# mittinatten/freesasa

Measured on AMD Instinct MI355X. Metric: atoms/sec SASA (L&R 20 slices), higher is better.
Workload: dtype f64

## Files before the change

### freesasa_amd/csrc/lr2_kernels.h

```cpp
#ifndef LR2_KERNELS_H
#define LR2_KERNELS_H

#include "sasa_kernels.h"

#ifdef SASA_EMU
namespace sasa_emu {
unsigned long long wave_ballot(bool p);
void wave_sync();
long long wave_exchange(long long v, int src);
}
#define LR2_BALLOT(p) sasa_emu::wave_ballot(p)
#define LR2_SYNC() sasa_emu::wave_sync()
#define LR2_SHFL(v, src) ((int)sasa_emu::wave_exchange((long long)(v), (src)))
#define LR2_POPC64(m) __builtin_popcountll(m)
#define LR2_POPC32(m) __builtin_popcount(m)
#define LR2_RANK(m, lane) __builtin_popcountll((m) & ((1ull << (lane)) - 1ull))
#define LR2_SHIFT_IN_LT1(w, c) (((w) << 1) | ((c) < 1.0 ? 1u : 0u))
#define LR2_SHIFT_IN_LT(w, v, lim) (((w) << 1) | ((v) < (lim) ? 1u : 0u))
#define LR2_UNIFORM(v) (v)
#define LR2_READLANE(v, src) LR2_SHFL((v), (src))
#define LR2_MUL24(a, b) ((int)(a) * (int)(b))
#define LR2_UMUL24(a, b) ((unsigned)(a) * (unsigned)(b))
#define LR2_RCPF(x) (1.0f / (x))
#define LR2_RSQF(x) (1.0f / sqrtf(x))
// ... 181 lines not shown
#define LR2_WARM(a, field) ((a).field)
#else
#define LR2_COLD(a, field) (*(const decltype(sasa::Lr2Args::field) *)lr2_cold_arg(offsetof(sasa::Lr2Args, field)))
#define LR2_WARM(a, field) LR2_COLD(a, field)
__device__ __forceinline__ const char *lr2_cold_arg(size_t off)
{
    auto p = __builtin_amdgcn_kernarg_segment_ptr();
    asm volatile("" : "+s"(p));
    return (const char *)p + off;
}
#endif

struct __attribute__((aligned(16))) Ab16 { double a, b; };
struct __attribute__((aligned(16))) Arc2 { double s, e; };

struct Lr2Layout {
    int o_atoms, o_ints, o_rec, o_mask, o_queue, o_tc, o_r2, o_tag, total;
};
SASA_HD int lr2_a16(int v) { return (v + 15) & ~15; }
SASA_HD int lr2_n_ints(int TA, int mw) { return 6 * TA + 1 + 8 + TA * mw; }
SASA_HD int lr2_n_row_ints(int TA) { return 9 * TA + 9 * TA + (9 * TA + 2); }
SASA_HD Lr2Layout lr2_layout(int TA, int ns, int pool, int mw, int ds)
{
    Lr2Layout L;
    const int items = TA * ns;
    int p = 0;
    L.o_atoms = p; p += 32 * TA + lr2_a16(8 * TA);
    L.o_ints = p;  p += lr2_a16(4 * lr2_n_ints(TA, mw));
    L.o_rec = p;   p += lr2_a16(24 * pool);
    L.o_mask = p;  p += lr2_a16(4 * items * mw);
    L.o_queue = p; p += lr2_a16(2 * items);
    L.o_tc = p;    p += lr2_a16(8 * items);
    if (p - L.o_rec < 32 * pool) p = L.o_rec + 32 * pool;
    int r2k = lr2_a16(8 * pool);
    if (r2k < lr2_a16(4 * lr2_n_row_ints(TA))) r2k = lr2_a16(4 * lr2_n_row_ints(TA));
    int r2 = r2k + lr2_a16(pool);
    const int r2q = lr2_a16(2 * items) + 256, r2s = 16 * LR2_LANES * (ds > 0 ? ds : 1);
    if (r2q > r2) r2 = r2q;
    if (r2s > r2) r2 = r2s;
    L.o_r2 = p;
    L.o_tag = p + r2k;
    p += r2;
    L.total = p;
    return L;
}

struct Lr2Mem {
    Quad *atom;
    double *adel;
    int *acell, *lead, *gsz, *acnt, *aoff, *sorig, *flags, *hist;
    unsigned *cmask;
    int *rowlo, *rinfo, *cpre;
    double *it_tc;
    unsigned *it_mask;
    unsigned short *queue;
    unsigned short *qtmp;
    Quad *hits;
    Ab16 *ab;
    double *beta;
    double *keys;
    unsigned char *tag;
    Arc2 *stack;
};

template <int SHAPE = 0>
SASA_D Lr2Mem lr2_carve(const Lr2Args &a, char *smem)
{
    const Lr2Layout L = lr2_layout(LR2_A_TA(a), LR2_A_NS(a), a.pool, LR2_A_MW(a), LR2_A_DS(a));
    const int TA = LR2_A_TA(a);
    Lr2Mem m;
    m.atom = (Quad *)(smem + L.o_atoms); m.adel = (double *)(smem + L.o_atoms + 32 * TA);
    int *q = (int *)(smem + L.o_ints);
    m.acell = q; q += TA; m.lead = q; q += TA; m.gsz = q; q += TA; m.acnt = q; q += TA; m.aoff = q; q += TA + 1;
    m.sorig = q; q += TA; m.flags = q; q += 8;
    m.cmask = (unsigned *)q;
    m.rowlo = (int *)(smem + L.o_r2); m.rinfo = m.rowlo + 9 * TA; m.cpre = m.rinfo + 9 * TA;
    m.it_tc = (double *)(smem + L.o_tc);
    m.it_mask = (unsigned *)(smem + L.o_mask);
    m.queue = (unsigned short *)(smem + L.o_queue);
    m.hits = (Quad *)(smem + L.o_rec);
    m.ab = (Ab16 *)(smem + L.o_rec);
    m.beta = (double *)(smem + L.o_rec + 16 * a.pool);
    m.keys = (double *)(smem + L.o_r2);
    m.tag = (unsigned char *)(smem + L.o_tag);
    m.hist = (int *)(smem + L.o_r2);
    m.qtmp = (unsigned short *)(smem + L.o_r2 + 256);
    m.stack = (Arc2 *)(smem + L.o_r2);
    return m;
}

SASA_D void lr2_record(double xd, double yd, double zd, double rj, double ri, double &ap, double &bp, double &Kout, double &d3sq, double &inv_d)
{
    const double D = xd * xd + yd * yd;
    double h;
    LR2_H2(D, h);
    const double inv = D > 0 ? 2.0 * h : 0x1p500;
    inv_d = D > 0 ? inv : 0.0;
    d3sq = D + zd * zd;
    const double K = (ri * ri - rj * rj) + d3sq;
    Kout = K;
    ap = -2.0 * zd * inv;
    bp = K * inv;
    if (!(D > 0) && zd == 0 && K == 0) bp = NAN;
}

SASA_D double lr2_arc_alpha(double t, const Ab16 &ab, double hh)
{
    const double v = fma(t, ab.a, ab.b);
    return acos_fast2_z(fma(fabs(v), -hh, 0.5), v);
}

struct Lr2Union {
    double ts, te, bs, be;
    int depth;
};
SASA_D void lr2_union_reset(Lr2Union &u) { u.ts = 0; u.te = -INFINITY; u.bs = 0; u.be = -INFINITY; u.depth = 0; }
SASA_D int lr2_med3(int v, int lo, int hi)
{
#ifdef SASA_EMU
    return v < lo ? lo : (v > hi ? hi : v);
#else
    int r;
    asm("v_med3_i32 %0, %1, %2, %3" : "=v"(r) : "v"(v), "s"(lo), "v"(hi));
    return r;
#endif
}
SASA_D Arc2 &lr2_level(Arc2 *stk, int depth, int ds)
{
    return (stk - 2 * LR2_LANES)[lr2_med3(depth, 2, ds > 0 ? ds + 1 : 2) * LR2_LANES];
}
SASA_D void lr2_union_step(double inf, double sup, Lr2Union &u, Arc2 *stk, int ds, int &maxd)
{
#ifdef LR2_UNION_SELECT
    const bool fresh = inf > u.te;
    const double mts = SASA_MIN(u.ts, inf), mte = SASA_MAX(u.te, sup);
    if (fresh) {
        Arc2 t; t.s = u.bs; t.e = u.be;
        lr2_level(stk, u.depth, ds) = t;
        u.bs = u.ts; u.be = u.te;
    }
    u.ts = fresh ? inf : mts;
    u.te = fresh ? sup : mte;
    u.depth += fresh ? 1 : 0;
    maxd = maxd > u.depth ? maxd : u.depth;
    while (u.be >= u.ts) {
        u.ts = SASA_MIN(u.ts, u.bs);
        --u.depth;
        if (u.depth >= 2) {
            const Arc2 lo = lr2_level(stk, u.depth, ds);
            u.bs = lo.s; u.be = lo.e;
        } else {
            u.be = -INFINITY;
        }
    }
#else
    if (inf > u.te) {
        Arc2 t; t.s = u.bs; t.e = u.be;
        lr2_level(stk, u.depth, ds) = t;
        u.bs = u.ts; u.be = u.te;
        u.ts = inf; u.te = sup;
        ++u.depth;
        maxd = maxd > u.depth ? maxd : u.depth;
    } else {
        u.ts = SASA_MIN(u.ts, inf);
        u.te = SASA_MAX(u.te, sup);
        while (u.be >= u.ts) {
            u.ts = SASA_MIN(u.ts, u.bs);
            --u.depth;
            if (u.depth >= 2) {
                const Arc2 lo = lr2_level(stk, u.depth, ds);
                u.bs = lo.s; u.be = lo.e;
            } else {
                u.be = -INFINITY;
            }
        }
    }
#endif
}

SASA_D double lr2_sweep(const Lr2Union &u, const Arc2 *stk, int ds)
{
    const int depth = u.depth;
    const bool two = depth >= 2;
    double s0 = two ? u.bs : u.ts;
    double e_below = two ? u.be : INFINITY;
    double sum = 0;
    if (depth > 2) {
        const Arc2 k0 = stk[0];
        s0 = k0.s;
        const double hi_ = s0 + SASA_TWOPI, lo_ = u.te - SASA_TWOPI;
        double pe = k0.e;
        for (int c = 1; c < depth - 2; ++c) {
            const Arc2 k = stk[(c < ds ? c : 0) * LR2_LANES];
            sum += SASA_MAX(SASA_MIN(k.s, hi_) - SASA_MAX(pe, lo_), 0.0);
            pe = k.e;
        }
        sum += SASA_MAX(SASA_MIN(u.bs, hi_) - SASA_MAX(pe, lo_), 0.0);
    }
    const double hi = s0 + SASA_TWOPI, lo = u.te - SASA_TWOPI;
    sum += SASA_MAX(SASA_MIN(u.ts, hi) - SASA_MAX(e_below, lo), 0.0);
    sum += SASA_MAX(hi - u.te, 0.0);
    return depth == 0 ? SASA_TWOPI : sum;
}

SASA_D double lr2_arc_kat(const double *arcs, const int *first, int k, Arc2 *stk, int ds)
{
    Lr2Union u;
    lr2_union_reset(u);
    int maxd = 0;
    for (int i = first[k]; i < first[k + 1]; ++i) lr2_union_step(arcs[2 * i], arcs[2 * i + 1], u, stk, ds, maxd);
    return maxd - 2 > ds ? NAN : lr2_sweep(u, stk, ds);
}

#ifndef LR2_NB_UNROLL
#ifndef LR2_ARC_STEPS
#define LR2_ARC_STEPS 2
#endif
#define LR2_NB_UNROLL 1
#endif
#define LR2_P1_G 3
#ifndef LR2_P1_G_COILS
#define LR2_P1_G_COILS LR2_P1_G
#endif
#define LR2_P1_G_OF(shape) ((shape) == 4 ? 4 : ((shape) == 1 ? LR2_P1_G_COILS : LR2_P1_G))
#define LR2_P1_HC(gs, g) ((g) == 4 ? ((gs) + 3) >> 2 : ((g) == 2 ? ((gs) + 1) >> 1 : lr2_div3((gs) + 2)))
#ifndef LR2_P1_ITEMS_MAX
#define LR2_P1_ITEMS_MAX 0x8000
#endif

SASA_D void lr2_overflow(const Lr2Args &a, int p0, int na, int err_code)
{
    int *const ovf_atoms = LR2_COLD(a, ovf_atoms), *const ovf_count = LR2_COLD(a, ovf_count);
    long long *const ovf_items = LR2_COLD(a, ovf_items);
    if (ovf_atoms) {
        const int w = SASA_ATOMIC_ADD_GLB(ovf_count, na);
        for (int k = 0; k < na; ++k) ovf_atoms[w + k] = p0 + k;
    } else if (ovf_items) {
        const int w = SASA_ATOMIC_ADD_GLB(ovf_count, 1);
        ovf_items[w] = (long long)p0 | ((long long)na << 32);
    } else {
        SASA_ATOMIC_MAX_GLB(&LR2_COLD(a, status)[ST_ERROR], err_code);
    }
}


SASA_D double lr2_slice_height(int s, double delta, double Ri) { return fma((double)s + 0.5, delta, -Ri); }
#ifndef LR2_WALK_Z
#define LR2_WALK_Z 1024.0
#endif
template <bool WALK>
SASA_D double lr2_slice_height_at(int s, double delta, double Ri, double zi)
{
    if (!WALK || !(fabs(zi) > LR2_WALK_Z)) return lr2_slice_height(s, delta, Ri);
    double z = (zi - Ri) - 0.5 * delta;
    for (int k = 0; k <= s; ++k) z += delta;
    return z - zi;
}

SASA_D unsigned lr2_tie12(double xd, double yd, double zd)
{
    unsigned long long a, b, c;
    memcpy(&a, &xd, 8); memcpy(&b, &yd, 8); memcpy(&c, &zd, 8);
    const unsigned h = (unsigned)a ^ ((unsigned)b * 0x9E3779B1u) ^ ((unsigned)c >> 7) ^ ((unsigned)c << 11);
    return (h ^ (h >> 13)) & 0xfffu;
}

#ifndef LR2_COVER_WANT
#define LR2_COVER_WANT 12
#endif
#define LR2_COVER_DENSITY 30
#ifndef LR2_COVER_MAX
#define LR2_COVER_MAX 20
#endif
SASA_D int lr2_cover_bin(double K, double d3sq, double ri)
{
    const float ct = (float)K * LR2_RSQF((float)d3sq) * LR2_RCPF(2.0f * (float)ri);
    const int b = (int)fmaf(ct, 10.0f, -2.0f);
    return b < 0 ? 0 : (b > 7 ? 7 : b);
}
SASA_D int lr2_cover_last_bin(unsigned long long h)
{
    int cum = 0, tb = 7;
    for (int b = 0; b < 8; ++b) {
        cum += (int)((h >> (8 * b)) & 255u);
        if (cum >= LR2_COVER_WANT && b < tb) tb = b;
    }
    return tb;
}
SASA_D double lr2_acos_lower(double c)
{
    const double c2 = c * c, k5 = c < 0 ? 0.075 : 0.17;
    return (1.5707963267948966 - 1e-9) - fma(c * c2, fma(k5, c2, 1.0 / 6.0), c);
}

#ifndef LR2_PRUNE
#define LR2_PRUNE 1
#endif
#ifndef LR2_PRUNE_ROUNDS
#define LR2_PRUNE_ROUNDS(pairs) ((pairs) ? 3 : 2)
#endif
#ifndef LR2_PRUNE_LIST
#define LR2_PRUNE_LIST 4
#endif
#define LR2_DEAD_TAG 0xff
struct __attribute__((aligned(16))) Lr2Cap { float x, y, z, c; };
SASA_HD int lr2_prune_arg(int want, int TA, int pool)
{
    if (8 * pool < (16 + 20 * LR2_PRUNE_LIST) * 2 * TA) return 0;
    return want > LR2_PRUNE_LIST ? LR2_PRUNE_LIST : (want < 0 ? 0 : want);
}
static inline int lr2_prune_want(int ns, bool dense) { return ns >= 32 ? 4 : (dense ? 0 : 3); }
SASA_D int lr2_cap_bin(float c) { const int b = (int)fmaf(c, 10.0f, -2.0f); return b < 0 ? 0 : (b > 7 ? 7 : b); }
template <int RMAX>
SASA_D void lr2_prune_contained(const Lr2Mem &m, int nh, int TA, int want, int lane)
{
    constexpr int LK = LR2_PRUNE_LIST;
    (void)want;
    unsigned long long *const chist = (unsigned long long *)m.keys;
    Lr2Cap *const bigc = (Lr2Cap *)(chist + 2 * TA);
    Lr2Cap *const bigs = bigc + 2 * LK * TA;
    int *const fill = m.acell;
    if (lane < 2 * TA) { chist[lane] = 0; fill[lane] = 0; }
    LR2_SYNC();
    float nx[RMAX], ny[RMAX], nz[RMAX], cc[RMAX];
    int lis[RMAX];
#define LR2_CAP_SIN(c) LR2_SQRTF(fmaf(-(c), (c), 1.0f + 4e-6f))
#define LR2_CAP_LIST(r, gp) ((gp) < nh && ny[r] != 0.0f && ny[r] == ny[r] ? 2 * (int)m.tag[gp] + (ny[r] > 0.0f ? 1 : 0) : -1)
    for (int r = 0; r < RMAX; ++r) {
        const int gp = lane + LR2_LANES * r;
        nx[r] = ny[r] = nz[r] = cc[r] = 0.0f;
        lis[r] = -1;
        if (gp < nh) {
            const Quad hq = m.hits[gp];
            const double ri = m.atom[(int)m.tag[gp]].w;
            const double d2 = hq.x * hq.x + hq.y * hq.y + hq.z * hq.z;
            const double K = (ri * ri - hq.w * hq.w) + d2;
            const float inv = LR2_RSQF((float)d2);
            nx[r] = (float)hq.x * inv; ny[r] = (float)hq.y * inv; nz[r] = (float)hq.z * inv;
            float c = (float)K * inv * LR2_RCPF(2.0f * (float)ri);
            c = c < -1.0f ? -1.0f : (c > 1.0f ? 1.0f : c);
            cc[r] = c;
            const int li = lis[r] = LR2_CAP_LIST(r, gp);
            if (li >= 0) LR2_ADD64_LDS(&chist[li], 1ull << (8 * lr2_cap_bin(c)));
        }
    }
    LR2_SYNC();
    if (lane < 2 * TA) {
        const unsigned long long h = chist[lane];
        const unsigned lo = (unsigned)h * 0x01010101u, hi = (unsigned)(h >> 32) * 0x01010101u + (lo >> 24) * 0x01010101u;
        const unsigned add = (unsigned)(127 - LK) * 0x01010101u;
        const unsigned mlo = (lo + add) & 0x80808080u, mhi = (hi + add) & 0x80808080u;
        const int tb = (mlo ? __builtin_ctz(mlo) >> 3 : (mhi ? 4 + (__builtin_ctz(mhi) >> 3) : 8)) - 1;
        chist[lane] = (unsigned long long)(long long)tb;
    }
    LR2_SYNC();
    for (int r = 0; r < RMAX; ++r) {
        const int li = lis[r];
        if (li < 0) continue;
        if (lr2_cap_bin(cc[r]) <= (int)chist[li]) {
            const int slot = SASA_ATOMIC_ADD_LDS(&fill[li], 1);
            if (slot < LK) {
                Lr2Cap q; q.x = nx[r]; q.y = ny[r]; q.z = nz[r]; q.c = cc[r];
                bigc[LK * li + slot] = q;
                ((float *)bigs)[LK * li + slot] = LR2_CAP_SIN(cc[r]);
            }
        }
    }
    LR2_SYNC();
    for (int r = 0; r < RMAX; ++r) {
        const int gp = lane + LR2_LANES * r;
        const int li = lis[r];
        if (li < 0) continue;
        const Lr2Cap *const L = bigc + LK * li;
        const float *const S = (const float *)bigs + LK * li;
        const float clim = cc[r] - 4e-6f, sj = LR2_CAP_SIN(cc[r]);
        bool inside = false;
        int nb = fill[li];
        nb = nb < LK ? nb : LK;
        for (int k = 0; k < nb; ++k) {
            const Lr2Cap q = L[k];
            const float dot = fmaf(nz[r], q.z, fmaf(ny[r], q.y, nx[r] * q.x));
            const float rhs = fmaf(sj, S[k], fmaf(cc[r], q.c, 8e-6f));
            inside = inside || (q.c <= clim && dot >= rhs);
        }
        if (inside) {
            m.tag[gp] = (unsigned char)LR2_DEAD_TAG;
            SASA_ATOMIC_ADD_LDS(&m.acnt[li >> 1], -1);
        }
    }
#undef LR2_CAP_LIST
#undef LR2_CAP_SIN
    LR2_SYNC();
}

struct Lr2Pre {
    int p0;
    long long rcf;
    int s0, s1;
    unsigned long long w0, w1;
    int rfl;
    Quad q;
    int cell, so;
};
SASA_D void lr2_pre_none(Lr2Pre &pre)
{
    pre.p0 = -1; pre.rcf = 0; pre.s0 = pre.s1 = 0; pre.w0 = pre.w1 = 0; pre.rfl = 1; pre.cell = 0; pre.so = 0;
    pre.q.x = pre.q.y = pre.q.z = 0; pre.q.w = 1;
}
template <int SHAPE>
SASA_D void lr2_pre_a(const Lr2Args &a, Lr2Pre &pre, int p0, int na, int lane)
{
    const int la = lr2_div9(lane);
    pre.p0 = p0;
    pre.rcf = LR2_WARM(a, s_idx)[p0 + (la < na ? la : na - 1)].cell;
}
template <int SHAPE>
SASA_D void lr2_pre_b(const Lr2Args &a, Lr2Pre &pre, int na, int lane)
{
    const int la = lr2_div9(lane), r = lane - 9 * la;
    const int c = (int)(pre.rcf & 0xffffffffLL), hw = (int)(pre.rcf >> 32);
    const int cprev = LR2_SHFL(c, lane >= 9 ? lane - 9 : lane);
    const int fl = hw & 63;
    int nx = (hw >> 6) & 8191, ny = (hw >> 19) & 8191;
    if (nx == 0) {
        const GridS *const g = LR2_COLD(a, grid) + LR2_COLD(a, s_idx)[pre.p0 + (la < na ? la : na - 1)].strct;
        nx = g->nx; ny = g->ny;
        SASA_OPAQUE(nx); SASA_OPAQUE(ny);
    }
    const int dz = lr2_div3(r < 9 ? r : 0) - 1, dy = (r < 9 ? r : 0) - 3 * (dz + 1) - 1;
    const bool out = (dy < 0 && (fl & CELL_Y0)) || (dy > 0 && (fl & CELL_Y1)) ||
                     (dz < 0 && (fl & CELL_Z0)) || (dz > 0 && (fl & CELL_Z1));
    const int row = out ? c : c + nx * (dy + ny * dz);
    const int x_lo = row - ((fl & CELL_X0) ? 0 : 1), x_hi = row + ((fl & CELL_X1) ? 0 : 1);
    const unsigned long long *const tbl = LR2_WARM(a, cell_tbl);
    if (tbl) {
        pre.s0 = x_lo; pre.s1 = x_hi + 1;
        pre.w0 = tbl[x_lo >> 5]; pre.w1 = tbl[(x_hi + 1) >> 5];
    } else {
        const int *const cell_start = LR2_COLD(a, cell_start);
        pre.s0 = cell_start[x_lo]; pre.s1 = cell_start[x_hi + 1];
    }
    pre.rfl = (out || la >= na ? 1 : 0) | (la == 0 || cprev != c ? 2 : 0);
}
template <int SHAPE>
SASA_D void lr2_pre_b2(const Lr2Args &a, Lr2Pre &pre)
{
    if (!LR2_WARM(a, cell_tbl)) return;
    const int *const first = LR2_WARM(a, cell_first);
    const int r0 = cell_rank(pre.w0, pre.s0), r1 = cell_rank(pre.w1, pre.s1);
    pre.s0 = first[r0]; pre.s1 = first[r1];
}
template <int SHAPE>
SASA_D void lr2_pre_c(const Lr2Args &a, Lr2Pre &pre, int na, int lane)
{
    const int p = pre.p0 + (lane < na ? lane : na - 1);
    pre.q = a.sq[p];
    const SortIdx si = LR2_WARM(a, s_idx)[p];
    pre.cell = lane < na ? (int)(si.cell & 0xffffffffLL) : -1 - lane;
    pre.so = si.orig;
}

template <int RMAX, bool COVER, bool PAIRS, int SHAPE, bool HOOKS, bool WALK>
SASA_D int lr2_tile(const Lr2Args &a, const Lr2Mem &m, int p0, int na, bool sample, bool tie_by_place, int lane_of_wave, int &wg_max_nn,
                    Lr2Pre &pre, int p0n, int nan, int &far_tiles)
{
    int lane = lane_of_wave;
    if (COVER) SASA_OPAQUE(lane);
    const int TA = LR2_A_TA(a), ns = LR2_A_NS(a), mw = LR2_A_MW(a);
    const int items = na * ns;
    LR2_MARK_BEGIN;
    LR2_COUNT(0, 1);

    if (pre.p0 != p0) {
        LR2_COUNT(11, 1);
        pre.p0 = p0;
        lr2_pre_c<SHAPE>(a, pre, na, lane);
        lr2_pre_a<SHAPE>(a, pre, p0, na, lane);
        lr2_pre_b<SHAPE>(a, pre, na, lane);
        lr2_pre_b2<SHAPE>(a, pre);
    }
    if (!HOOKS && (!WALK || !a.work_items) && LR2_BALLOT(lane < na && fabs(pre.q.z) > LR2_WALK_Z) != 0) {
        ++far_tiles;
        if (!WALK) {
            lr2_pre_none(pre);
            return 3;
        }
    }
    if (lane < TA) {
        Quad q = pre.q;
        if (lane >= na) { q.x = q.y = q.z = 0; q.w = 1; }
        const double del = lane < na ? lr2_div_ns(2 * q.w, (double)ns, LR2_WARM(a, inv_ns)) : 0.0;
        m.atom[lane] = q; m.adel[lane] = del; m.sorig[lane] = lane < na ? pre.so : 0;
        m.acnt[lane] = 0;
        m.gsz[lane] = 0;
    }
    if (lane < 8) m.flags[lane] = 0;
    unsigned lm;
    {
        const int cprev = LR2_SHFL(pre.cell, lane > 0 ? lane - 1 : 0);
        lm = (unsigned)LR2_BALLOT(lane < na && (lane == 0 || pre.cell != cprev));
    }
    int lo = 0, my_cnt = 0, info = 0;
    {
        const int la = lr2_div9(lane);
        if (la < na && (pre.rfl & 3) == 2) {
            const unsigned above = lm >> (la + 1);
            const int gs = (above ? la + 1 + __builtin_ctz(above) : na) - la, hc = LR2_P1_HC(gs, LR2_P1_G_OF(SHAPE));
            lo = pre.s0;
            my_cnt = LR2_MUL24(pre.s1 - pre.s0, hc);
            info = la | (gs << 4) | (hc << 8) | ((hc == 1 ? 0x20000 : (hc == 2 ? 0x10000 : 0xaaab)) << 10);
        }
    }
    lr2_pre_none(pre);
    const unsigned long long rm = LR2_BALLOT(my_cnt > 0);
    const int incl = lr2_scan_add(my_cnt, lane);
    const int nrows = LR2_POPC64(rm);
    const int total_c = LR2_READLANE(incl, LR2_LANES - 1);
    if (lane == 0) m.cpre[0] = 0;
    if (my_cnt > 0) {
        const int ri = LR2_RANK(rm, lane);
        m.cpre[ri + 1] = incl; m.rowlo[ri] = lo; m.rinfo[ri] = info;
    }
    LR2_SYNC();
    if (total_c >= LR2_P1_ITEMS_MAX) { LR2_COUNT(9, 1); return 1; }

    LR2_STOP(0);
    LR2_MARK(0);
    int nh = 0;
    {
        const int per = (total_c + LR2_LANES - 1) / LR2_LANES;
        const int f = lane * per;
        const int fend = f + per < total_c ? f + per : total_c;
        int t = 0;
        int c_lo = 0, c_hi = 0, rl = 0, ri_ = 0;
        if (f < total_c) {
            for (int step = 32; step >= 1; step >>= 1)
                if (t + step <= nrows - 1 && m.cpre[t + step] <= f) t += step;
            c_lo = m.cpre[t]; c_hi = m.cpre[t + 1]; rl = m.rowlo[t]; ri_ = m.rinfo[t];
        }
        constexpr int P1_G = LR2_P1_G_OF(SHAPE);
        LR2_COUNT(3, (per + LR2_NB_UNROLL - 1) / LR2_NB_UNROLL * LR2_NB_UNROLL * P1_G);
        for (int base = 0; base < per; base += LR2_NB_UNROLL) {
            int q[LR2_NB_UNROLL], la0[LR2_NB_UNROLL], two[LR2_NB_UNROLL];
            double x[LR2_NB_UNROLL], y[LR2_NB_UNROLL], z[LR2_NB_UNROLL], rq[LR2_NB_UNROLL];
            for (int j = 0; j < LR2_NB_UNROLL; ++j) {
                const int fj = f + base + j;
                const bool live = fj < fend;
                if (live && fj >= c_hi) {
                    ++t;
                    c_lo = c_hi; c_hi = m.cpre[t + 1]; rl = m.rowlo[t]; ri_ = m.rinfo[t];
                }
                const int lead = ri_ & 15, gs = (ri_ >> 4) & 15, hc = (ri_ >> 8) & 3;
                const unsigned i = (unsigned)(fj - c_lo) & 0x7fffu;
                const unsigned c = LR2_UMUL24(i, (unsigned)ri_ >> 10) >> 17;
                const int h = (int)i - LR2_MUL24(c, hc);
                const int left = gs - P1_G * h;
                q[j] = live ? rl + (int)c : -1;
                la0[j] = live ? lead + P1_G * h : 0;
                two[j] = live ? (left < P1_G ? left : P1_G) : 0;
            }
            for (int j = 0; j < LR2_NB_UNROLL; ++j) {
                const unsigned u = (unsigned)(q[j] < 0 ? 0 : q[j]);
                { const Quad v = a.sq[u]; x[j] = v.x; y[j] = v.y; z[j] = v.z; rq[j] = v.w; }
            }
            for (int g = 0; g < P1_G; ++g) {
                bool hit[LR2_NB_UNROLL];
                double dx[LR2_NB_UNROLL], dy[LR2_NB_UNROLL], dz[LR2_NB_UNROLL];
                Quad ai[LR2_NB_UNROLL];
                for (int j = 0; j < LR2_NB_UNROLL; ++j) ai[j] = m.atom[la0[j] + (g < two[j] ? g : 0)];
                for (int j = 0; j < LR2_NB_UNROLL; ++j) {
                    const double cut2 = (ai[j].w + rq[j]) * (ai[j].w + rq[j]);
                    dx[j] = x[j] - ai[j].x; dy[j] = y[j] - ai[j].y; dz[j] = z[j] - ai[j].z;
                    const double d2 = dx[j] * dx[j] + dy[j] * dy[j] + dz[j] * dz[j];
                    hit[j] = (g < two[j]) & (q[j] != p0 + la0[j] + g) & (d2 < cut2);
                }
                for (int j = 0; j < LR2_NB_UNROLL; ++j) {
                    const unsigned long long hm = LR2_BALLOT(hit[j]);
                    if (hit[j]) {
                        const int la = la0[j] + g;
                        int slot = nh + LR2_RANK(hm, lane);
                        slot = slot < a.pool ? slot : a.pool - 1;
                        Quad hq; hq.x = dx[j]; hq.y = dy[j]; hq.z = dz[j]; hq.w = rq[j];
                        m.hits[slot] = hq;
                        m.tag[slot] = (unsigned char)la;
                        if (!(HOOKS && (a.hooks & 2))) {
                            LR2_INC_LDS(&m.acnt[la]);
                        } else {
                            const int sa = SASA_ATOMIC_ADD_LDS(&m.acnt[la], 1);
                            const int cap = LR2_COLD(a, nb_cap);
                            if (sa < cap) LR2_COLD(a, nb_out)[(size_t)m.sorig[la] * cap + sa] = LR2_COLD(a, s_idx)[q[j]].orig;
                        }
                    }
                    nh += LR2_POPC64(hm);
                }
            }
        }
    }
    LR2_SYNC();

    LR2_STOP(1);
    LR2_MARK(1);
    if (HOOKS && (a.hooks & 1)) {
        if (lane < na) LR2_COLD(a, nn_out)[m.sorig[lane]] = m.acnt[lane];
        LR2_SYNC();
        return 0;
    }
    bool ovf;
    int nn_max;
    {
        const int c = lane < TA ? m.acnt[lane] : 0, pc = (c + 1) & ~1;
        const int incl = lr2_scan_add(pc, lane), cmax = lr2_scan_max16(c, lane);
        if (lane < TA) m.aoff[lane] = incl - pc;
        if (lane == TA - 1) m.aoff[TA] = incl;
        const int total = LR2_READLANE(incl, TA - 1);
        nn_max = LR2_READLANE(cmax, TA - 1);
        ovf = nn_max > 32 * mw || total > a.pool || nh > a.pool || nh > LR2_LANES * RMAX;
        if (lane == 0) {
            if (nn_max > wg_max_nn) wg_max_nn = nn_max;
            if (sample) {
                const int need = total / hist_bin_width(TA);
                SASA_ATOMIC_ADD_GLB(&LR2_COLD(a, status)[ST_HIST + (need < 63 ? need : 63)], 1);
            }
        }
    }
    LR2_SYNC();
    if (ovf) { LR2_COUNT(9, 1); return 1; }
    LR2_STOP(2);
    if (LR2_PRUNE && !HOOKS) {
        const int pk = LR2_COLD(a, prune);
        constexpr int PR = RMAX < LR2_PRUNE_ROUNDS(PAIRS) ? RMAX : LR2_PRUNE_ROUNDS(PAIRS);
        if (pk > 0 && nh > 0 && nh <= LR2_LANES * PR) {
            lr2_prune_contained<PR>(m, nh, TA, pk, lane);
            const int c = lane < TA ? m.acnt[lane] : 0, pc = (c + 1) & ~1;
            const int incl = lr2_scan_add(pc, lane), cmax = lr2_scan_max16(c, lane);
            if (lane < TA) m.aoff[lane] = incl - pc;
            if (lane == TA - 1) m.aoff[TA] = incl;
            nn_max = LR2_READLANE(cmax, TA - 1);
            LR2_SYNC();
        }
    }
    LR2_STOP(15);
    const int mwt = (nn_max + 31) >> 5;
    const bool cover = COVER && a.cover > 0 && nh >= LR2_MUL24(a.cover, na);

    LR2_MARK(2);
    {
        double r_a[RMAX], r_b[RMAX], r_beta[RMAX], r_key[RMAX];
        int r_pos[RMAX];
        int r_cb[RMAX];
        unsigned low = 0xfffu;
        SASA_OPAQUE(low);
        unsigned long long *const chist = (unsigned long long *)m.acell;
        const bool bk = cover && ns * mw >= 16;
        int *const bh = (int *)m.it_mask;
        if (cover) {
            if (lane < TA) chist[lane] = 0;
            LR2_SYNC();
        }
        for (int r = 0; r < RMAX; ++r) {
            const int gp = lane + LR2_LANES * r;
            r_pos[r] = -1;
            r_cb[r] = 0;
            if (gp < nh) {
                const Quad hq = m.hits[gp];
                const int la = (int)m.tag[gp];
                if (la == LR2_DEAD_TAG) continue;
                const int sa = SASA_ATOMIC_ADD_LDS(&m.gsz[la], 1);
                const int o = m.aoff[la];
                const double ri = m.atom[la].w;
                double Kc, d3sq, inv_d;
                r_pos[r] = o | (m.acnt[la] << 16);
                lr2_record(hq.x, hq.y, hq.z, hq.w, ri, r_a[r], r_b[r], Kc, d3sq, inv_d);
                r_beta[r] = atan2_inv(hq.y, hq.x, inv_d) + SASA_PI;
                if (r_b[r] != r_b[r]) LR2_OR_LDS((unsigned *)&m.flags[6], 1u << la);
                r_key[r] = lr_rank_key(r_beta[r], tie_by_place ? (unsigned)sa : lr2_tie12(hq.x, hq.y, hq.z), low);
                if (!bk) m.keys[o + sa] = r_key[r];
                r_cb[r] = la << 3;
                if (cover) {
                    const int b = lr2_cover_bin(Kc, d3sq, ri);
                    r_cb[r] |= b;
                    LR2_ADD64_LDS(&chist[la], 1ull << (8 * b));
                }
            }
        }
        if (lane < TA && (m.acnt[lane] & 1)) m.keys[m.aoff[lane] + m.acnt[lane]] = INFINITY;
        if (!cover && lane < TA) m.lead[lane] = 0;
        LR2_SYNC();
        if (cover) {
            const unsigned long long h = lane < TA ? chist[lane] : 0;
            LR2_SYNC();
            if (lane < TA) {
                m.gsz[lane] = lr2_cover_last_bin(h);
                m.acell[lane] = 0;
                m.lead[lane] = 0;
                for (int w = 0; w < mw; ++w) m.cmask[LR2_MUL24(lane, mw) + w] = 0;
            }
            LR2_SYNC();
        }
        if (bk) {
            for (int q = lane; q < 16 * TA; q += LR2_LANES) bh[q] = 0;
            LR2_SYNC();
            for (int r = 0; r < RMAX; ++r) {
                if (r_pos[r] < 0) continue;
                int b = (int)(r_key[r] * (16.0 / SASA_TWOPI));
                b = b < 0 ? 0 : (b > 15 ? 15 : b);
                const int idx = SASA_ATOMIC_ADD_LDS(&bh[((r_cb[r] >> 3) & 7) * 16 + b], 1);
                r_cb[r] |= (b << 6) | (idx << 10);
            }
            LR2_SYNC();
            for (int q0 = 0; q0 < 16 * TA; q0 += LR2_LANES) {
                const int q = q0 + lane, v = q < 16 * TA ? bh[q] : 0;
                const int incl = lr2_scan_add16(v, lane);
                LR2_SYNC();
                if (q < 16 * TA) bh[q] = incl - v;
            }
            LR2_SYNC();
            for (int r = 0; r < RMAX; ++r) {
                if (r_pos[r] < 0) continue;
                const int first = bh[((r_cb[r] >> 3) & 7) * 16 + ((r_cb[r] >> 6) & 15)];
                m.keys[(r_pos[r] & 0xffff) + first + ((r_cb[r] >> 10) & 0xff)] = r_key[r];
            }
            LR2_SYNC();
        }
        int cnt_rank_[RMAX] = {0}; (void)cnt_rank_;
        for (int r = 0; r < RMAX; ++r) {
            if (r_pos[r] < 0) continue;
            const int o = r_pos[r] & 0xffff, nn = r_pos[r] >> 16;
            const double kme = r_key[r];
            int rank = 0, t = 0;
            if (bk) {
                const int la_ = (r_cb[r] >> 3) & 7, b = (r_cb[r] >> 6) & 15;
                const int lo = bh[la_ * 16 + b], hi = b < 15 ? bh[la_ * 16 + b + 1] : m.acnt[la_];
                rank = lo;
                for (int q = lo; q < hi; ++q) rank += m.keys[o + q] < kme ? 1 : 0;
                t = nn;
#ifdef SASA_EMU
                cnt_rank_[r] = hi - lo;
#endif
            }
            for (; t + 4 <= nn; t += 4) {
                const Arc2 k0 = *(const Arc2 *)(m.keys + o + t), k1 = *(const Arc2 *)(m.keys + o + t + 2);
                rank += k0.s < kme ? 1 : 0;
                rank += k0.e < kme ? 1 : 0;
                rank += k1.s < kme ? 1 : 0;
                rank += k1.e < kme ? 1 : 0;
            }
            for (; t < nn; t += 2) {
                const Arc2 kk = *(const Arc2 *)(m.keys + o + t);
                rank += kk.s < kme ? 1 : 0;
                rank += kk.e < kme ? 1 : 0;
            }
            Ab16 rc; rc.a = r_a[r]; rc.b = r_b[r];
            m.ab[o + rank] = rc;
            m.beta[o + rank] = r_beta[r];
            SASA_ATOMIC_ADD_LDS(&m.lead[(r_cb[r] >> 3) & 7], rank);
            if (cover) {
                const int la = (r_cb[r] >> 3) & 7;
                if ((r_cb[r] & 7) <= m.gsz[la] && SASA_ATOMIC_ADD_LDS(&m.acell[la], 1) < LR2_COVER_MAX)
                    LR2_OR_LDS(&m.cmask[LR2_MUL24(la, mw) + (rank >> 5)], 1u << (rank & 31));
            }
        }
#ifdef SASA_EMU
        if (bk) for (int r = 0; r < RMAX; ++r) LR2_COUNT_LANES(4, 5, cnt_rank_[r]);
#endif
        if (lane < TA && (m.acnt[lane] & 1)) {
            int zero = 0; SASA_OPAQUE(zero);
            Ab16 rc; rc.a = (double)zero; rc.b = 1e300;
            m.ab[m.aoff[lane] + m.acnt[lane]] = rc;
            m.beta[m.aoff[lane] + m.acnt[lane]] = rc.a;
        }
    }
    LR2_SYNC();
    {
        const int nn_ = lane < TA ? m.acnt[lane] : 0;
        const bool twice = lane < TA && m.lead[lane] != ((LR2_MUL24(nn_, nn_) - nn_) >> 1);
        if (LR2_BALLOT(twice) != 0) return 2;
    }

    LR2_STOP(3);
    LR2_MARK(3);
    lr2_pre_a<SHAPE>(a, pre, p0n, nan, lane);
    const float inv_ns = LR2_RCPF((float)ns);
#ifndef LR2_ARC_BALANCED
#define LR2_ARC_BALANCED 1
#endif
#ifndef LR2_SCREEN5
#define LR2_SCREEN5 1
#endif
#if defined(SASA_EMU) && defined(LR2_EMU_DUMP)
    const bool direct = false;
#else
    const bool direct = LR2_ARC_BALANCED && COVER && !PAIRS && items <= LR2_LANES;
#endif
    int dcnt = 0;
    if (!direct) {
        m.hist[lane] = 0;
        LR2_SYNC();
    }
    int cnt_filter_[2] = {0, 0}, cnt_filter_k_ = 0, cnt_screen_ = 0; (void)cnt_filter_; (void)cnt_filter_k_; (void)cnt_screen_;
    auto finish_item = [&](int it, int la, double t, double h2, double Ri, int o, int cnt, bool buried, bool circle) -> int {
        double area = 0;
        if (buried || !circle) cnt = 0;
        else if (cnt == 0) area = m.adel[la] * Ri * SASA_TWOPI;
        if (cover && circle) {
            double cts = 0, cte = -INFINITY;
            for (int wi = 0; wi < mwt; ++wi) {
                unsigned wc = cnt > 0 ? (m.it_mask[LR2_MUL24(it, mw) + wi] & m.cmask[LR2_MUL24(la, mw) + wi]) : 0u;
                const int R = o + 32 * wi;
                while (wc != 0) {
                    const int q = R + __builtin_ctz(wc);
                    wc &= wc - 1;
#ifdef SASA_EMU
                    ++cnt_filter_[cnt_filter_k_ & 1];
#endif
                    const Ab16 ab = m.ab[q];
                    const double bt = m.beta[q];
                    const double c = fma(t, ab.a, ab.b) * h2;
                    const double al = lr2_acos_lower(c);
                    const double inf = bt - al, sup = bt + al;
                    const bool fresh = inf > cte;
                    const double nts = fresh ? inf : SASA_MIN(cts, inf), nte = fresh ? sup : SASA_MAX(cte, sup);
                    if (c <= 0.9) { cts = nts; cte = nte; }
                }
            }
            if (cte - cts >= SASA_TWOPI) cnt = 0;
        }
#ifdef SASA_EMU
        ++cnt_filter_k_;
#endif
        m.it_tc[it] = cnt == 0 ? area : 0.5 * h2;
        if (direct) return cnt;
        unsigned short qt = 0xffff;
        if (cnt > 0) {
            const int bin = 63 - (cnt < 63 ? cnt : 63);
            const int ord = SASA_ATOMIC_ADD_LDS(&m.hist[bin], 1);
            qt = (unsigned short)((bin << 10) | ord);
        }
        m.qtmp[it] = qt;
        return cnt;
    };
    const int hp = (ns + 1) >> 1;
    if (PAIRS) {
        int ln = lane;
        SASA_OPAQUE(ln);
        if (ln < LR2_MUL24(na, hp)) {
            int la = (int)(((float)ln + 0.5f) * LR2_RCPF((float)hp)), j = ln - LR2_MUL24(la, hp);
            if (j < 0) { --la; j += hp; } else if (j >= hp) { ++la; j -= hp; }
            const int sa_ = 2 * j, it0 = LR2_MUL24(la, ns) + sa_;
            const bool second = sa_ + 1 < ns;
            const double Ri = m.atom[la].w, del = m.adel[la];
            const double zi_ = WALK ? m.atom[la].z : 0.0;
            const double t0 = lr2_slice_height_at<WALK>(sa_, del, Ri, zi_), t1 = lr2_slice_height_at<WALK>(second ? sa_ + 1 : sa_, del, Ri, zi_);
            const double A0 = Ri * Ri - t0 * t0, A1 = Ri * Ri - t1 * t1;
            const bool circ0 = A0 > 0, circ1 = second && A1 > 0;
            double h0, h1;
            LR2_H2(circ0 ? A0 : 1.0, h0);
            LR2_H2(circ1 ? A1 : 1.0, h1);
            const double T0 = lr2_arc_limit(circ0 ? A0 : 1.0, h0), T1 = lr2_arc_limit(circ1 ? A1 : 1.0, h1);
            const int o = m.aoff[la], nn = m.aoff[la + 1] - o;
            double vmin0 = 0.0, vmin1 = 0.0;
            int cnt0 = 0, cnt1 = 0;
            for (int wi = 0; wi < mwt; ++wi) {
                unsigned w0 = 0, w1 = 0;
                const int k1 = nn - 32 * wi < 32 ? nn - 32 * wi : 32;
                const Ab16 *R = m.ab + (o + 32 * wi);
                int k = k1 - 2;
                if (k1 > 0 && (k1 & 2)) {
                    const Ab16 ra = R[k], rb = R[k + 1];
                    const double c0 = fma(t0, ra.a, ra.b), c1 = fma(t0, rb.a, rb.b);
                    const double d0 = fma(t1, ra.a, ra.b), d1 = fma(t1, rb.a, rb.b);
                    vmin0 = SASA_MIN(vmin0, SASA_MIN(c0, c1));
                    vmin1 = SASA_MIN(vmin1, SASA_MIN(d0, d1));
                    w0 = LR2_SHIFT_IN_LT(w0, c1, T0); w0 = LR2_SHIFT_IN_LT(w0, c0, T0);
                    w1 = LR2_SHIFT_IN_LT(w1, d1, T1); w1 = LR2_SHIFT_IN_LT(w1, d0, T1);
                    k -= 2;
                }
                for (; k >= 0; k -= 4) {
                    const Ab16 r2 = R[k], r3 = R[k + 1], r0 = R[k - 2], r1 = R[k - 1];
                    const double c2 = fma(t0, r2.a, r2.b), c3 = fma(t0, r3.a, r3.b);
                    const double c0 = fma(t0, r0.a, r0.b), c1 = fma(t0, r1.a, r1.b);
                    const double d2 = fma(t1, r2.a, r2.b), d3 = fma(t1, r3.a, r3.b);
                    const double d0 = fma(t1, r0.a, r0.b), d1 = fma(t1, r1.a, r1.b);
                    vmin0 = SASA_MIN(SASA_MIN(vmin0, c0), SASA_MIN(c1, SASA_MIN(c2, c3)));
                    vmin1 = SASA_MIN(SASA_MIN(vmin1, d0), SASA_MIN(d1, SASA_MIN(d2, d3)));
                    w0 = LR2_SHIFT_IN_LT(w0, c3, T0); w0 = LR2_SHIFT_IN_LT(w0, c2, T0); w0 = LR2_SHIFT_IN_LT(w0, c1, T0); w0 = LR2_SHIFT_IN_LT(w0, c0, T0);
                    w1 = LR2_SHIFT_IN_LT(w1, d3, T1); w1 = LR2_SHIFT_IN_LT(w1, d2, T1); w1 = LR2_SHIFT_IN_LT(w1, d1, T1); w1 = LR2_SHIFT_IN_LT(w1, d0, T1);
                }
                m.it_mask[LR2_MUL24(it0, mw) + wi] = w0;
                cnt0 += LR2_POPC32(w0);
                if (second) {
                    m.it_mask[LR2_MUL24(it0 + 1, mw) + wi] = w1;
                    cnt1 += LR2_POPC32(w1);
                }
            }
            finish_item(it0, la, t0, circ0 ? h0 : 0.0, Ri, o, cnt0, vmin0 <= -T0, circ0);
            if (second) finish_item(it0 + 1, la, t1, circ1 ? h1 : 0.0, Ri, o, cnt1, vmin1 <= -T1, circ1);
        }
    } else if (LR2_SCREEN5 && SHAPE == 2) {
        constexpr int Q = 5, G = 100 / Q;
        int ln = lane;
        SASA_OPAQUE(ln);
        if (ln < LR2_MUL24(na, G)) {
            int la = (int)(((float)ln + 0.5f) * (1.0f / (float)G)), j = ln - LR2_MUL24(la, G);
            if (j < 0) { --la; j += G; } else if (j >= G) { ++la; j -= G; }
            const int s0 = Q * j, it0 = LR2_MUL24(la, ns) + s0;
            const double Ri = m.atom[la].w, del = m.adel[la];
            const double zi_ = WALK ? m.atom[la].z : 0.0;
            double t[Q], T[Q], vmin[Q];
            int cnt[Q];
            for (int q = 0; q < Q; ++q) {
                t[q] = lr2_slice_height_at<WALK>(s0 + q, del, Ri, zi_);
                const double A = Ri * Ri - t[q] * t[q];
                double hq;
                LR2_H2(A > 0 ? A : 1.0, hq);
                T[q] = lr2_arc_limit(A > 0 ? A : 1.0, hq);
                vmin[q] = 0.0;
                cnt[q] = 0;
            }
            const int o = m.aoff[la], nn = m.aoff[la + 1] - o;
            for (int wi = 0; wi < mwt; ++wi) {
                unsigned w[Q];
                for (int q = 0; q < Q; ++q) w[q] = 0;
                const int k1 = nn - 32 * wi < 32 ? nn - 32 * wi : 32;
                const Ab16 *R = m.ab + (o + 32 * wi);
                Ab16 rn = R[k1 > 0 ? k1 - 1 : 0];
                for (int k = k1 - 1; k >= 0; --k) {
                    const Ab16 ra = rn;
                    rn = R[k > 0 ? k - 1 : 0];
                    for (int q = 0; q < Q; ++q) {
                        const double c = fma(t[q], ra.a, ra.b);
                        vmin[q] = SASA_MIN(vmin[q], c);
                        w[q] = LR2_SHIFT_IN_LT(w[q], c, T[q]);
                    }
                }
                for (int q = 0; q < Q; ++q) {
                    m.it_mask[LR2_MUL24(it0 + q, mw) + wi] = w[q];
                    cnt[q] += LR2_POPC32(w[q]);
                }
            }
            for (int q = 0; q < Q; ++q) {
                const double A = Ri * Ri - t[q] * t[q];
                double hq;
                LR2_H2(A > 0 ? A : 1.0, hq);
                finish_item(it0 + q, la, t[q], A > 0 ? hq : 0.0, Ri, o, cnt[q], vmin[q] <= -T[q], A > 0);
            }
        }
    } else
    for (int it = lane; it < items; it += LR2_LANES) {
        int la = (int)(((float)it + 0.5f) * inv_ns), s = it - LR2_MUL24(la, ns);
        if (s < 0) { --la; s += ns; } else if (s >= ns) { ++la; s -= ns; }
        const double Ri = m.atom[la].w, t = lr2_slice_height_at<WALK>(s, m.adel[la], Ri, WALK ? m.atom[la].z : 0.0);
        const double A = Ri * Ri - t * t;
        double h2 = 0;
        int cnt = 0, o = 0;
        bool buried = false;
        if (A > 0) {
            LR2_H2(A, h2);
            const double T = lr2_arc_limit(A, h2);
            o = m.aoff[la];
            const int nn = m.aoff[la + 1] - o;
            double vmin = 0.0;
            for (int wi = 0; wi < mwt; ++wi) {
                unsigned w = 0;
                const int k1 = nn - 32 * wi < 32 ? nn - 32 * wi : 32;
                const Ab16 *R = m.ab + (o + 32 * wi);
                int k = k1 - 2;
                if (k1 > 0 && (k1 & 2)) {
                    const double c0 = fma(t, R[k].a, R[k].b), c1 = fma(t, R[k + 1].a, R[k + 1].b);
                    vmin = SASA_MIN(vmin, c0);
// ... 558 lines not shown
```

Before: 1.082 billion.

## Compact pruned hits in LDS instead of tagging them dead

After the containment prune, surviving hits are compacted in place using ballot and rank, and the new count is returned. Later loops then iterate only over live hits instead of skipping dead-tagged entries. The histogram threshold logic is moved into a helper that also saturates byte counts above the list size before the prefix sums. Compaction adds a sync per round and extra LDS traffic, which may or may not pay off against skipped work.

```diff
diff --git a/freesasa_amd/csrc/lr2_kernels.h b/freesasa_amd/csrc/lr2_kernels.h
--- a/freesasa_amd/csrc/lr2_kernels.h
+++ b/freesasa_amd/csrc/lr2_kernels.h
@@ -507,7 +507,6 @@
 #ifndef LR2_PRUNE_LIST
 #define LR2_PRUNE_LIST 4
 #endif
-#define LR2_DEAD_TAG 0xff
 struct __attribute__((aligned(16))) Lr2Cap { float x, y, z, c; };
 SASA_HD int lr2_prune_arg(int want, int TA, int pool)
 {
@@ -516,8 +515,21 @@
 }
 static inline int lr2_prune_want(int ns, bool dense) { return ns >= 32 ? 4 : (dense ? 0 : 3); }
 SASA_D int lr2_cap_bin(float c) { const int b = (int)fmaf(c, 10.0f, -2.0f); return b < 0 ? 0 : (b > 7 ? 7 : b); }
+SASA_HD int lr2_prune_last_bin(unsigned long long h)
+{
+    constexpr int LK = LR2_PRUNE_LIST;
+    constexpr unsigned long long ones = 0x0101010101010101ull;
+    const unsigned long long big = (((h & (0xf8ull * ones)) >> 1) + 0x7cull * ones) & (0x80ull * ones);
+    const unsigned long long gt = (((h & (0x07ull * ones)) + (0x7full - (LK + 1)) * ones) & (0x80ull * ones)) | big;
+    const unsigned long long m8 = (gt >> 7) * 0xffull;
+    h = (h & ~m8) | ((unsigned long long)(LK + 1) * ones & m8);
+    const unsigned lo = (unsigned)h * 0x01010101u, hi = (unsigned)(h >> 32) * 0x01010101u + (lo >> 24) * 0x01010101u;
+    const unsigned add = (unsigned)(127 - LK) * 0x01010101u;
+    const unsigned mlo = (lo + add) & 0x80808080u, mhi = (hi + add) & 0x80808080u;
+    return (mlo ? __builtin_ctz(mlo) >> 3 : (mhi ? 4 + (__builtin_ctz(mhi) >> 3) : 8)) - 1;
+}
 template <int RMAX>
-SASA_D void lr2_prune_contained(const Lr2Mem &m, int nh, int TA, int want, int lane)
+SASA_D int lr2_prune_contained(const Lr2Mem &m, int nh, int TA, int want, int lane)
 {
     constexpr int LK = LR2_PRUNE_LIST;
     (void)want;
@@ -550,14 +562,7 @@
         }
     }
     LR2_SYNC();
-    if (lane < 2 * TA) {
-        const unsigned long long h = chist[lane];
-        const unsigned lo = (unsigned)h * 0x01010101u, hi = (unsigned)(h >> 32) * 0x01010101u + (lo >> 24) * 0x01010101u;
-        const unsigned add = (unsigned)(127 - LK) * 0x01010101u;
-        const unsigned mlo = (lo + add) & 0x80808080u, mhi = (hi + add) & 0x80808080u;
-        const int tb = (mlo ? __builtin_ctz(mlo) >> 3 : (mhi ? 4 + (__builtin_ctz(mhi) >> 3) : 8)) - 1;
-        chist[lane] = (unsigned long long)(long long)tb;
-    }
+    if (lane < 2 * TA) chist[lane] = (unsigned long long)(long long)lr2_prune_last_bin(chist[lane]);
     LR2_SYNC();
     for (int r = 0; r < RMAX; ++r) {
         const int li = lis[r];
@@ -572,30 +577,47 @@
         }
     }
     LR2_SYNC();
+    unsigned kept = 0;
+#pragma unroll
     for (int r = 0; r < RMAX; ++r) {
         const int gp = lane + LR2_LANES * r;
         const int li = lis[r];
-        if (li < 0) continue;
-        const Lr2Cap *const L = bigc + LK * li;
-        const float *const S = (const float *)bigs + LK * li;
-        const float clim = cc[r] - 4e-6f, sj = LR2_CAP_SIN(cc[r]);
         bool inside = false;
-        int nb = fill[li];
-        nb = nb < LK ? nb : LK;
-        for (int k = 0; k < nb; ++k) {
-            const Lr2Cap q = L[k];
-            const float dot = fmaf(nz[r], q.z, fmaf(ny[r], q.y, nx[r] * q.x));
-            const float rhs = fmaf(sj, S[k], fmaf(cc[r], q.c, 8e-6f));
-            inside = inside || (q.c <= clim && dot >= rhs);
-        }
-        if (inside) {
-            m.tag[gp] = (unsigned char)LR2_DEAD_TAG;
-            SASA_ATOMIC_ADD_LDS(&m.acnt[li >> 1], -1);
-        }
+        if (li >= 0) {
+            const Lr2Cap *const L = bigc + LK * li;
+            const float *const S = (const float *)bigs + LK * li;
+            const float clim = cc[r] - 4e-6f, sj = LR2_CAP_SIN(cc[r]);
+            int nb = fill[li];
+            nb = nb < LK ? nb : LK;
+            for (int k = 0; k < nb; ++k) {
+                const Lr2Cap q = L[k];
+                const float dot = fmaf(nz[r], q.z, fmaf(ny[r], q.y, nx[r] * q.x));
+                const float rhs = fmaf(sj, S[k], fmaf(cc[r], q.c, 8e-6f));
+                inside = inside || (q.c <= clim && dot >= rhs);
+            }
+            if (inside) SASA_ATOMIC_ADD_LDS(&m.acnt[li >> 1], -1);
+        }
+        if (gp < nh && !inside) kept |= 1u << r;
+    }
+    int nk = 0;
+#pragma unroll
+    for (int r = 0; r < RMAX; ++r) {
+        const int gp = lane + LR2_LANES * r;
+        const bool keep = (kept >> r) & 1u;
+        const unsigned long long km = LR2_BALLOT(keep);
+        const int dst = nk + LR2_RANK(km, lane);
+        const bool move = keep && dst != gp;
+        double hx = 0, hy = 0, hz = 0, hw = 0;
+        int tg = 0;
+        if (move) { const Quad q = m.hits[gp]; hx = q.x; hy = q.y; hz = q.z; hw = q.w; tg = m.tag[gp]; }
+        LR2_SYNC();
+        if (move) { Quad q; q.x = hx; q.y = hy; q.z = hz; q.w = hw; m.hits[dst] = q; m.tag[dst] = (unsigned char)tg; }
+        nk += LR2_POPC64(km);
     }
 #undef LR2_CAP_LIST
 #undef LR2_CAP_SIN
     LR2_SYNC();
+    return nk;
 }
 
 struct Lr2Pre {
@@ -831,11 +853,12 @@
     LR2_SYNC();
     if (ovf) { LR2_COUNT(9, 1); return 1; }
     LR2_STOP(2);
+    int nr = nh;
     if (LR2_PRUNE && !HOOKS) {
         const int pk = LR2_COLD(a, prune);
         constexpr int PR = RMAX < LR2_PRUNE_ROUNDS(PAIRS) ? RMAX : LR2_PRUNE_ROUNDS(PAIRS);
         if (pk > 0 && nh > 0 && nh <= LR2_LANES * PR) {
-            lr2_prune_contained<PR>(m, nh, TA, pk, lane);
+            nr = lr2_prune_contained<PR>(m, nh, TA, pk, lane);
             const int c = lane < TA ? m.acnt[lane] : 0, pc = (c + 1) & ~1;
             const int incl = lr2_scan_add(pc, lane), cmax = lr2_scan_max16(c, lane);
             if (lane < TA) m.aoff[lane] = incl - pc;
@@ -866,10 +889,9 @@
             const int gp = lane + LR2_LANES * r;
             r_pos[r] = -1;
             r_cb[r] = 0;
-            if (gp < nh) {
+            if (gp < nr) {
                 const Quad hq = m.hits[gp];
                 const int la = (int)m.tag[gp];
-                if (la == LR2_DEAD_TAG) continue;
                 const int sa = SASA_ATOMIC_ADD_LDS(&m.gsz[la], 1);
                 const int o = m.aoff[la];
                 const double ri = m.atom[la].w;
```

Result: faster. 1.102 billion (median of 6 runs) (+1.9%).
